# OpenDriveLab/ThinkTwice

Hardware: AMD Instinct MI355X
Metric: frames/sec forward (4-cam+LiDAR, thinktwice.py cfg) (higher is better)
Workload: dtype bf16x3h; 1 GPU; forward_inference thinktwice.py cfg: 8 frames x (2 sweeps x 4 cams x 448x896 + 65536-pt LiDAR), ResNet50+PAFPN+DepthNet+UNet+LSS splat, LidarNet, fusion, 5-stage decoder; parallelism=replicas x1 (no data-path collective), launch=eager launches, 3 batches in flight on alternating streams, batches_in_flight=3

## Files before the change

### thinktwice_amd/csrc/conv_choose.cpp

```cpp
#include <stdint.h>

#include "conv_choose.h"

namespace tt {
namespace {

bool aligned16(const void* p) { return (reinterpret_cast<uintptr_t>(p) & 15) == 0; }

void set_tile(ConvChoice* c, int family, int bn, int waves_m, int waves_n, int bkb, int stages) {
    c->family = family;
    c->bn = bn;
    c->waves_m = waves_m;
    c->waves_n = waves_n;
    c->bkb = bkb;
    c->stages = stages;
}

bool choose_h2(const ConvArgs& a, ConvChoice* c) {
    if (a.gather || a.m_dev || a.ws || a.pixel_shuffle2 || a.Cin % 64 != 0 || a.KH * a.KW > 31 || a.K < 64) return false;
    static const bool pipe = env_flag("TT_H2_PIPE", true);
    if (pipe && a.Cout % 128 == 0 && a.K >= 1152) set_tile(c, CONV_H2_PIPE, 128, 4, 1, 128, 32);
    else if (a.Cout > 64) set_tile(c, CONV_H2, 128, 4, 2, 128, 32);
    else set_tile(c, CONV_H2, 64, 8, 1, 128, 33);
    return true;
}

bool choose_small(const ConvArgs& a, ConvChoice* c) {
    if (a.gather || a.m_dev || a.M > 4096) return false;
    if ((long long)div_up(a.M, 32) * div_up(a.Cout, 32) > 4096) return false;
    set_tile(c, CONV_SMALL, 32, 1, 1, 32, 1);
    return true;
}

int tail_split_rows(const ConvArgs& a) {
    if (a.Cout % 256 != 0) return 0;
    const int tiles_m = div_up(a.M, 256), tiles_n = a.Cout / 256;
    const long long T = (long long)tiles_m * tiles_n;
    const int rounds = (int)((T + kNumCU - 1) / kNumCU);
    const int last = (int)(T - (long long)kNumCU * (rounds - 1));
    if (rounds < 2 || rounds > 8 || last > kNumCU / 4) return 0;
    const int peel = div_up(last, tiles_n);
    return peel < tiles_m ? tiles_m - peel : 0;
}

bool choose_x3_splitk(const ConvArgs& a, bool assume_ws, ConvChoice* c) {
    if (a.gather || a.m_dev || a.M < 512 || a.M > 8192 || a.Cout < 64 || a.KH * a.KW > 32) return false;
    if (a.Cin % 32 != 0 || a.K < 1024 || a.pixel_shuffle2) return false;
    const int tiles = div_up(a.M, 256) * div_up(a.Cout, 64);
    const int nk = a.K / 32;
    if (tiles >= 256) return false;
    int sp = 512 / tiles;
    if (sp > nk / 8) sp = nk / 8;
    if (sp > 16) sp = 16;
    if (sp < 2) return false;
    const int slices = div_up(nk, div_up(nk, sp));
    if (slices < 2 || (!assume_ws && a.ws_slices < slices)) return false;
    set_tile(c, CONV_GLDS, 64, 8, 1, 128, 2);
    c->x3 = true;
    c->splits = sp;
    c->slices = slices;
    return true;
}

bool choose_sp_runs(const ConvArgs& a, ConvChoice* c) {
    if (!a.gather || a.row_perm || a.KH != 1 || a.KW != 27) return false;
    if (a.stride != 1) return false;
    if (a.Cin % 32 != 0 || a.Cin > 128 || a.M < 2048 || a.pixel_shuffle2) return false;
    if ((a.in_cstride & 3) || (a.in_coff & 3)) return false;
    if (a.Cout == 32) set_tile(c, CONV_SP_RUNS, 32, 8, 1, 128, 2);
    else if (a.Cout == 64) set_tile(c, CONV_SP_RUNS, 64, 8, 1, 128, 2);
    else if (a.Cout == 128) set_tile(c, CONV_SP_RUNS, 128, 4, 2, 128, 2);
    else return false;
    c->gather = c->x3 = true;
    return true;
}

bool x3_pipe_ok(const ConvArgs& a, int bn) {
    return !(a.gather || a.m_dev || (bn != 256 && bn != 128) || a.Cout % bn != 0 || a.Cin % 32 != 0 || a.KH * a.KW > 31 || a.K < 64);
}

bool choose_x3(const ConvArgs& a, ConvChoice* c) {
    c->x3 = true;
    if (a.gather) {
        if (choose_sp_runs(a, c)) return true;
        const bool cin_ok = a.Cin >= 16 && (a.Cin & (a.Cin - 1)) == 0;
        if (!cin_ok || a.M < 2048 || a.Cout < 16 || a.Cout > 128) return false;
        set_tile(c, CONV_GLDS, a.Cout <= 32 ? 32 : (a.Cout <= 64 ? 64 : 128), 8, 1, 128, 2);
        c->gather = true;
        return true;
    }
    if (a.m_dev || a.M < 2048 || a.KH * a.KW > 32) return false;
    if (a.Cin % 32 != 0 || a.K < 64) return false;
    const bool apair = (a.flags & 32) != 0;
    if (apair && (a.in_coff % 16 != 0 || a.in_cstride % 16 != 0)) return false;
    c->apair = apair;
    if (a.Cout < 64) {
        if (a.Cout > 32 || a.Cout < 8) return false;
        if (!apair && a.M < (1 << 16)) return false;
        set_tile(c, CONV_GLDS, 32, 8, 1, 128, 2);
        return true;
    }
    const int tiles_m = div_up(a.M, 256);
    auto cost = [&](int bn, double rate) {
        const long long tiles = (long long)tiles_m * div_up(a.Cout, bn);
        return (double)((tiles + kNumCU - 1) / kNumCU) * bn / rate;
    };
    const bool wide = a.Cout % 256 == 0 || a.Cout > 512;
    const int main_rows = tail_split_rows(a);
    auto cost256 = [&]() {
        if (!main_rows) return cost(256, 1.0);
        const long long tn = a.Cout / 256;
        const long long main_tiles = (long long)main_rows * tn, tail_tiles = (long long)(tiles_m - main_rows) * tn * 4;
        return (double)((main_tiles + kNumCU - 1) / kNumCU) * 256 / 1.0 + (double)((tail_tiles + kNumCU - 1) / kNumCU) * 64 / 0.63;
    };
    const double c256 = wide ? cost256() : 1e30;
    const double c128 = a.Cout > 64 ? cost(128, (a.K >= 1152 && a.Cout % 128 == 0) ? 0.95 : 0.85) : 1e30;
    const double c64 = cost(64, 0.63);
    const int bn = (c256 <= c128 && c256 <= c64) ? 256 : (c128 <= c64 ? 128 : 64);
    static const bool pipe = env_flag("TT_X3_PIPE", true);
    if (pipe && a.K >= 1152 && bn != 64 && x3_pipe_ok(a, bn)) {
        static const bool run3 = env_flag("TT_X3_RUN3", true);
        const bool runs = run3 && a.KW == 3 && a.KH <= 5 && a.stride == 1 && a.dil == 1 && a.pad == 1 && a.OH == a.H && a.OW == a.W &&
                          (a.N == 1 || a.in_nstride == (long long)a.H * a.W * a.in_cstride);
        set_tile(c, runs ? CONV_X3_RUN3 : CONV_X3_PIPE, bn, 4, 1, 128, 23);
    } else if (bn == 256) {
        set_tile(c, CONV_GLDS, 256, 4, 2, 128, 23);
    } else {
        set_tile(c, CONV_GLDS, bn, 8, 1, 128, 2);
    }
    if (bn == 256) c->main_rows = main_rows;
    return true;
}

bool choose_glds(const ConvArgs& a, int dtype, ConvChoice* c) {
    constexpr int min_tiles = 2;
    if (a.gather) {
        const bool cin_ok = a.Cin >= 16 && (a.Cin & (a.Cin - 1)) == 0;
        if (dtype == TT_F32 || !cin_ok || a.M < 2048 || a.Cout < 16 || a.Cout > 128) return false;
        if (a.Cout <= 32) set_tile(c, CONV_GLDS, 32, 8, 1, 128, 2);
        else if (a.Cout <= 64) set_tile(c, CONV_GLDS, 64, 8, 1, 128, 2);
        else set_tile(c, CONV_GLDS, 128, 4, 2, 128, 2);
        c->gather = true;
        return true;
    }
    if (a.m_dev || a.M < 2048 || a.Cout < 64 || a.KH * a.KW > 32) return false;
    if (dtype == TT_F32) {
        if (a.Cin % 16 != 0 || div_up(a.K, 16) < min_tiles) return false;
        if (a.Cout > 64) set_tile(c, CONV_GLDS, 128, 4, 2, 64, 3);
        else set_tile(c, CONV_GLDS, 64, 8, 1, 64, 3);
        return true;
    }
    if (a.Cin % 32 != 0 || div_up(a.K, 32) < min_tiles) return false;
    if (a.Cout > 64) {
        const long long tiles256 = (long long)div_up(a.M, 256) * (a.Cout / 256);
        if (a.Cout % 256 == 0 && tiles256 >= 200) {
            if (a.Cin % 64 == 0) {
                set_tile(c, CONV_GLDS, 256, 2, 4, 128, 2);
                c->main_rows = tail_split_rows(a);
            } else {
                set_tile(c, CONV_GLDS, 256, 2, 4, 64, 3);
            }
        } else if (a.K <= 512) {
            set_tile(c, CONV_GLDS, 128, 2, 2, 64, 3);
        } else {
            set_tile(c, CONV_GLDS, 128, 4, 2, 64, 3);
        }
        return true;
    }
    if (a.Cin % 64 == 0) set_tile(c, CONV_GLDS, 64, 8, 1, 128, 2);
    else set_tile(c, CONV_GLDS, 64, 8, 1, 64, 3);
    return true;
}

int choose_igemm(const ConvArgs& a, int dtype, bool ws, bool assume_ws, ConvChoice* c) {
    if (a.Cout > 64) set_tile(c, CONV_IGEMM, 128, 2, 2, 64, 2);
    else if (a.Cout > 32) set_tile(c, CONV_IGEMM, 64, 2, 2, 64, 2);
    else set_tile(c, CONV_IGEMM, 32, 4, 1, 64, 2);
    if (dtype != TT_F32) c->bkb = 128;
    c->gather = a.gather != nullptr;
    const int tiles = div_up(a.M, 128) * div_up(a.Cout, c->bn);
    const int nk = div_up(a.K, c->bkb / (dtype == TT_F32 ? 4 : 2));
    if (ws && !a.m_dev && tiles < 128 && nk >= 8) {
        int sp = div_up(512, tiles);
        if (sp > nk / 2) sp = nk / 2;
        if (sp > 64) sp = 64;
        c->splits = sp < 1 ? 1 : sp;
    }
    if (c->splits <= 1) return 0;
    c->slices = c->splits;
    if (!assume_ws) {
        c->slices = 0;
        if (a.ws_slices > 0) {
            const int eff = div_up(nk, div_up(nk, c->splits));
            TT_REQUIRE(a.ws_slices >= eff, "tt_conv2d_fwd: split-K workspace holds %d slices, %d needed", a.ws_slices, eff);
            c->slices = eff;
        }
    }
    return 0;
}

}

int conv_choose(const ConvArgs& a, const ConvFacts& f, ConvChoice* c) {
    *c = ConvChoice{};
    c->splits = 1;
    const bool ws = a.ws || f.assume_ws;
    if (f.weight_h2) {
        TT_REQUIRE(aligned16(f.weight_h2), "tt_conv2d_fwd: weight_h2 must be 16-byte aligned");
        TT_REQUIRE(choose_h2(a, c), "tt_conv2d_fwd: weight_h2 layer outside the h2 kernel's contract (Cin=%d KH*KW=%d)", a.Cin,
                   a.KH * a.KW);
        return 0;
    }
    TT_REQUIRE(!f.out2 || a.vec_epi, "tt_conv2d_fwd: out2 needs the vector epilogue (aligned channel counts)");
    TT_REQUIRE(!f.res1_up || a.vec_epi, "tt_conv2d_fwd: an upsampled res1 needs the vector epilogue (aligned channel counts)");
    TT_REQUIRE(!f.res1_f32 || (a.vec_epi && a.res_vec), "tt_conv2d_fwd: an f32 res1 needs the vector epilogue and aligned residual rows");
    TT_REQUIRE(!(f.dtype == TT_F32 && a.out_dtype != TT_F32 && a.res1) || (a.vec_epi && a.res_vec),
               "tt_conv2d_fwd: a 16-bit output of an f32 layer with a residual needs the vector epilogue");
    if (a.flags & (32 | 64)) {
        TT_REQUIRE(a.vec_epi && aligned16(f.weight_x3) && a.K % 16 == 0,
                   "tt_conv2d_fwd: in_pair / out_pair need the vector epilogue and a 16-byte aligned weight_x3");
        TT_REQUIRE(choose_x3(a, c), "tt_conv2d_fwd: pair-format layer outside the LDS-DMA bf16x3 kernel's contract (M=%d Cin=%d Cout=%d)",
                   a.M, a.Cin, a.Cout);
        return 0;
    }
    if (!ws && !f.out2 && !f.res1_up && !f.res1_f32 && choose_small(a, c)) return 0;
    const bool x3 = f.weight_x3 && f.dtype == TT_F32;
    if (ws && x3 && a.K % 16 == 0 && aligned16(f.weight_x3) && choose_x3_splitk(a, f.assume_ws, c)) return 0;
    if (!ws && x3) {
        TT_REQUIRE(aligned16(f.weight_x3) && a.K % 16 == 0, "tt_conv2d_fwd: weight_x3 needs 16-byte alignment and K %% 16 == 0 (K = %d)",
                   a.K);
        if (choose_x3(a, c)) return 0;
        *c = ConvChoice{};
        c->splits = 1;
    }
    if (!ws && choose_glds(a, f.dtype, c)) return 0;
    return choose_igemm(a, f.dtype, ws, f.assume_ws, c);
}

ConvChoice conv_tail_choice(const ConvChoice& c) {
    ConvChoice t{};
    set_tile(&t, CONV_GLDS, 64, 8, 1, 128, 2);
    t.x3 = c.x3;
    t.apair = c.apair;
    t.splits = 1;
    return t;
}

void conv_label(const ConvChoice& c, int dtype, char* out, size_t bytes) {
    const char* tn = dtype == TT_F32 ? "float" : "16-bit";
    const char* pre = c.apair ? " pre-split A" : "";
    const char* tail = c.main_rows > 0 ? " + tail" : "";
    switch (c.family) {
        case CONV_H2: snprintf(out, bytes, "conv_h2_kernel<%d, %d, %d, %d, %d>", c.bn, c.waves_m, c.waves_n, c.stages / 10, c.stages % 10); break;
        case CONV_H2_PIPE: snprintf(out, bytes, "conv_h2_pipe_kernel"); break;
        case CONV_SMALL: snprintf(out, bytes, "conv_small_kernel"); break;
        case CONV_SP_RUNS: snprintf(out, bytes, "sp_conv_runs_kernel<%d, %d, %d>", c.bn / (32 * c.waves_n), c.waves_m, c.waves_n); break;
        case CONV_X3_PIPE: snprintf(out, bytes, "conv_x3_pipe_kernel<%s>%s%s", c.bn == 128 ? "4, 1, 128" : "4, 1", pre, tail); break;
        case CONV_X3_RUN3: snprintf(out, bytes, "conv_x3_run3_kernel<%d>%s%s", c.bn, pre, tail); break;
        case CONV_GLDS:
            snprintf(out, bytes, "conv_igemm_glds_kernel<%s, %d, %d, %d, %d, %d, %s, %s>%s%s", tn, c.bn, c.waves_m, c.waves_n, c.bkb,
                     c.stages, c.gather ? "true" : "false", c.x3 ? "true" : "false", pre, c.splits > 1 ? " split-K" : tail);
            break;
        default: snprintf(out, bytes, "conv_igemm_kernel<%s, 128, %d>%s", tn, c.bn, c.splits > 1 ? " split-K" : ""); break;
    }
}

}
```

### thinktwice_amd/csrc/conv_choose.h

```cpp
#pragma once
#include <stddef.h>

#include "tt_common.h"

namespace tt {

struct ConvArgs {
    const void* in;
    const void* weight;
    void* out;
    const float* scale;
    const float* shift;
    const float* shift_n;
    const void* res1;
    const void* res2;
    const int* gather;
    const int* m_dev;
    const int* row_perm;
    const unsigned* row_mask;
    float* ws;
    long long in_nstride, out_nstride;
    int N, H, W, Cin, in_cstride, in_coff;
    int Cout, KH, KW, stride, pad, dil;
    int OH, OW, out_cstride, out_coff;
    int pixel_shuffle2, shift_n_mod;
    int res1_cstride, res1_coff, res2_cstride, res2_coff;
    int act, out_dtype;
    int M, K;
    int cin_fast;
    int out_fast;
    int vec_epi;
    int res_vec;
    int splits;
    int tiles_n;
    int m_begin;
    int ws_slices;
    int flags;
    int res1_up_h, res1_up_w;
    float* out2;
    int out2_cstride, out2_coff;
    long long* trace;
};

enum ConvFamily {
    CONV_H2,
    CONV_H2_PIPE,
    CONV_SMALL,
    CONV_SP_RUNS,
    CONV_X3_PIPE,
    CONV_X3_RUN3,
    CONV_GLDS,
    CONV_IGEMM,
};

struct ConvFacts {
    int dtype;
    const void* weight_x3;
    const void* weight_h2;
    bool out2, res1_up, res1_f32;
    bool assume_ws;
};

struct ConvChoice {
    int family;
    int bn;
    int waves_m, waves_n, bkb, stages;
    bool gather, x3, apair;
    int main_rows;
    int splits;
    int slices;
};

int conv_choose(const ConvArgs& a, const ConvFacts& f, ConvChoice* c);
ConvChoice conv_tail_choice(const ConvChoice& c);
void conv_label(const ConvChoice& c, int dtype, char* out, size_t bytes);

}
```

### thinktwice_amd/csrc/conv_common.h

```cpp
#pragma once
#include <type_traits>
#include "conv_choose.h"

namespace tt {
extern thread_local char g_conv_kernel[96];
extern long long* g_conv_trace;


typedef float f32x16 __attribute__((ext_vector_type(16)));
typedef __bf16 bf16x8 __attribute__((ext_vector_type(8)));
typedef _Float16 f16x8 __attribute__((ext_vector_type(8)));

template <typename T> struct Mfma;
template <> struct Mfma<float> {
    __device__ static __forceinline__ void run(const uint4& a, const uint4& b, f32x16& c) {
        c = __builtin_amdgcn_mfma_f32_32x32x2f32(__uint_as_float(a.x), __uint_as_float(b.x), c, 0, 0, 0);
        c = __builtin_amdgcn_mfma_f32_32x32x2f32(__uint_as_float(a.y), __uint_as_float(b.y), c, 0, 0, 0);
        c = __builtin_amdgcn_mfma_f32_32x32x2f32(__uint_as_float(a.z), __uint_as_float(b.z), c, 0, 0, 0);
        c = __builtin_amdgcn_mfma_f32_32x32x2f32(__uint_as_float(a.w), __uint_as_float(b.w), c, 0, 0, 0);
    }
};
template <> struct Mfma<uint16_t> {
    __device__ static __forceinline__ void run(const uint4& a, const uint4& b, f32x16& c) {
        c = __builtin_amdgcn_mfma_f32_32x32x16_bf16(__builtin_bit_cast(bf16x8, a),
// ... 89 lines not shown
            v[4] += u.b.x; v[5] += u.b.y; v[6] += u.b.z; v[7] += u.b.w;
        } else {
            v[0] += u.x; v[1] += u.y; v[2] += u.z; v[3] += u.w;
        }
    };
    auto add_rv = [&](float (&v)[CO], const RV& u) {
        if constexpr (sizeof(T) == 2 && CO == 8) {
            const uint32_t w[4] = {u.x, u.y, u.z, u.w};
#pragma unroll
            for (int e = 0; e < 4; ++e) {
                float a, b;
                Pair16<T>::unpack(w[e], a, b);
                v[2 * e] += a; v[2 * e + 1] += b;
            }
        } else if constexpr (sizeof(T) == 2) {
            const uint32_t w[2] = {u.x, u.y};
#pragma unroll
            for (int e = 0; e < 2; ++e) {
                float a, b;
                Pair16<T>::unpack(w[e], a, b);
                v[2 * e] += a; v[2 * e + 1] += b;
            }
        } else {
            add_rvf(v, u);
        }
    };
    const bool r1_f32 = EXT && sizeof(T) == 2 && (p.flags & 128) != 0;
    const bool fast_act = (act == TT_ACT_NONE || act == TT_ACT_RELU);
    const bool r1_up = EXT && p.res1_up_w > 0;
    auto res1_row = [&](int m) -> long long {
        if (!r1_up) return (long long)m;
        const int n = m / ohw, rem = m - n * ohw;
        const int oh = rem / p.OW, ow = rem - oh * p.OW;
        return ((long long)n * p.res1_up_h + (oh * p.res1_up_h) / p.OH) * p.res1_up_w + (ow * p.res1_up_w) / p.OW;
    };
    auto out_offset = [&](int m, int cc, int& n) -> long long {
        if (p.out_fast) {
            if (has_sn) n = m / ohw;
            return (long long)m * p.out_cstride + p.out_coff + cc;
        }
        n = m / ohw;
        const int rem = m - n * ohw;
        int oh = rem / p.OW, ow = rem - oh * p.OW;
        int OWo = p.OW;
        if (p.pixel_shuffle2) {
            oh = 2 * oh + (q >> 1);
            ow = 2 * ow + (q & 1);
            OWo = 2 * p.OW;
        }
        return (long long)n * p.out_nstride + ((long long)oh * OWo + ow) * p.out_cstride + p.out_coff + cc;
    };
    const bool nt_store = (p.flags & 16) != 0;
    auto store_row = [&](long long o, const float (&v)[CO]) {
        if constexpr (CO == 4) {
            typedef float f4v __attribute__((ext_vector_type(4)));
            if (nt_store) __builtin_nontemporal_store(f4v{v[0], v[1], v[2], v[3]}, reinterpret_cast<f4v*>(reinterpret_cast<float*>(p.out) + o));
            else *reinterpret_cast<float4*>(reinterpret_cast<float*>(p.out) + o) = make_float4(v[0], v[1], v[2], v[3]);
        } else if (sizeof(T) == 4 && (p.flags & 64)) {
            uint4 hi, lo;
            uint32_t* hp = reinterpret_cast<uint32_t*>(&hi);
            uint32_t* lp = reinterpret_cast<uint32_t*>(&lo);
#pragma unroll
            for (int e = 0; e < 4; ++e) {
                const uint32_t h = pack_bf16x2(v[2 * e], v[2 * e + 1]);
                hp[e] = h;
                lp[e] = pack_bf16x2(v[2 * e] - __uint_as_float(h << 16), v[2 * e + 1] - __uint_as_float(h & 0xffff0000u));
            }
            float* g = reinterpret_cast<float*>(p.out) + (o & ~15ll) + ((o & 8) ? 4 : 0);
            *reinterpret_cast<uint4*>(g) = hi;
            *reinterpret_cast<uint4*>(g + 8) = lo;
        } else {
            uint4 pk;
            if constexpr (sizeof(T) == 2) {
                pk.x = Pair16<T>::pack(v[0], v[1]);
                pk.y = Pair16<T>::pack(v[2], v[3]);
                pk.z = Pair16<T>::pack(v[4], v[5]);
                pk.w = Pair16<T>::pack(v[6], v[7]);
            } else if (p.out_dtype == TT_F16) {
                pk.x = pack_f16x2(v[0], v[1]);
                pk.y = pack_f16x2(v[2], v[3]);
                pk.z = pack_f16x2(v[4], v[5]);
                pk.w = pack_f16x2(v[6], v[7]);
            } else {
                pk.x = pack_bf16x2(v[0], v[1]);
                pk.y = pack_bf16x2(v[2], v[3]);
                pk.z = pack_bf16x2(v[4], v[5]);
                pk.w = pack_bf16x2(v[6], v[7]);
            }
            *reinterpret_cast<uint4*>(reinterpret_cast<uint16_t*>(p.out) + o) = pk;
        }
    };
    float* const out2 = (EXT && p.out2) ? p.out2 + p.out2_coff + co : nullptr;
    auto store_row2 = [&](long long row, const float (&v)[CO]) {
        typedef float f4v __attribute__((ext_vector_type(4)));
        float* q2 = out2 + row * p.out2_cstride;
#pragma unroll
        for (int e = 0; e < CO; e += 4)
            __builtin_nontemporal_store(f4v{v[e], v[e + 1], v[e + 2], v[e + 3]}, reinterpret_cast<f4v*>(q2 + e));
    };
    const int cc = col_ok ? co : 0;
#pragma unroll
    for (int i = 0; i < TM; ++i) {
        const int mb = m0 + wm * WTM + i * 32;
        const int last_row = (mb + 31 < Mlim ? mb + 31 : Mlim - 1);
        const int img = mb / ohw;
        const bool one_image = (img == last_row / ohw);
        const bool sn_folded = has_sn && one_image;
        const bool sn_loop = has_sn && !sn_folded;
        float shb[TN];
#pragma unroll
        for (int j = 0; j < TN; ++j) shb[j] = sh[j];
        if (sn_folded) {
            const int nimg = img % p.shift_n_mod;
#pragma unroll
            for (int j = 0; j < TN; ++j) {
                const int cj = n0 + wn * WTN + j * 32 + (lane & 31);
                if (cj < p.Cout) shb[j] += p.shift_n[(long long)nimg * cout_real + cj % cout_real];
            }
        }
        stage_scaled<TN, WTN>(sC, acc[i], sc, shb, lane);
        const bool full_block = (mb + 32 <= Mlim) && (n0 + wn * WTN + WTN <= p.Cout);
        const bool out_linear = p.out_fast || (one_image && !p.pixel_shuffle2);
        const long long obase = (p.out_fast ? 0 : (long long)img * (p.out_nstride - (long long)ohw * p.out_cstride)) +
                                p.out_coff + co;
        if (fast_act && rvec && out_linear && !sn_loop && !has_r2 && full_block) {
            auto hot = [&](auto mode_c) {
                constexpr int RM = decltype(mode_c)::value;
                constexpr bool R1 = RM != 0;
                using R1T = typename std::conditional<RM == 2, RVF, RV>::type;
                using RES = typename std::conditional<RM == 2, float, T>::type;
                constexpr int PG = (sizeof(R1T) > 16 && NPASS > 4) ? 4 : (NPASS > 8 ? 8 : NPASS);
#pragma unroll
                for (int g0 = 0; g0 < NPASS; g0 += PG) {
                    R1T r1[R1 ? PG : 1];
                    int mrow[PG];
#pragma unroll
                    for (int q = 0; q < PG; ++q) {
                        const int m = mb + (g0 + q) * rpp + row_in_pass;
                        mrow[q] = p.row_perm ? p.row_perm[m] : m;
                    }
                    if constexpr (R1) {
#pragma unroll
                        for (int q = 0; q < PG; ++q)
                            r1[q] = *reinterpret_cast<const R1T*>(reinterpret_cast<const RES*>(p.res1) +
                                                                 res1_row(mrow[q]) * p.res1_cstride + p.res1_coff + co);
                    }
#pragma unroll
                    for (int q = 0; q < PG; ++q) {
                        const int rl = (g0 + q) * rpp + row_in_pass;
                        const int mr = mrow[q];
                        float v[CO];
#pragma unroll
                        for (int e = 0; e < CO; e += 4) {
                            const float4 t0 = *reinterpret_cast<const float4*>(sC + rl * LDC + col_l + e);
                            v[e] = t0.x; v[e + 1] = t0.y; v[e + 2] = t0.z; v[e + 3] = t0.w;
                        }
                        if constexpr (RM == 2) add_rvf(v, r1[q]);
                        else if constexpr (RM == 1) add_rv(v, r1[q]);
                        if (act == TT_ACT_RELU) {
#pragma unroll
                            for (int e = 0; e < CO; ++e) v[e] = v[e] > 0.f ? v[e] : 0.f;
                        }
                        store_row((long long)mr * p.out_cstride + obase, v);
                        if (out2) store_row2(mr, v);
                    }
                }
            };
            if (!has_r1) hot(std::integral_constant<int, 0>{});
            else if (EXT && sizeof(T) == 2 && r1_f32) {
                if constexpr (EXT && sizeof(T) == 2) hot(std::integral_constant<int, 2>{});
            } else hot(std::integral_constant<int, 1>{});
        } else {
#pragma unroll 1
            for (int pass = 0; pass < NPASS; ++pass) {
                const int rl = pass * rpp + row_in_pass;
                const int m = mb + rl;
                if (m >= Mlim || !col_ok) continue;
                float v[CO];
#pragma unroll
                for (int e = 0; e < CO; e += 4) {
                    const float4 t0 = *reinterpret_cast<const float4*>(sC + rl * LDC + col_l + e);
                    v[e] = t0.x; v[e + 1] = t0.y; v[e + 2] = t0.z; v[e + 3] = t0.w;
                }
                int n = 0;
                const int mo = p.row_perm ? p.row_perm[m] : m;
                const long long o = out_offset(mo, co, n);
                if (sn_loop) {
                    const float* sn = p.shift_n + (long long)(n % p.shift_n_mod) * cout_real + co;
#pragma unroll
                    for (int e = 0; e < CO; ++e) v[e] += sn[e];
                }
#pragma unroll
                for (int which = 0; which < 2; ++which) {
                    const void* rb = which ? p.res2 : p.res1;
                    if (!rb) continue;
                    const T* rp = reinterpret_cast<const T*>(rb) +
                                  (which ? (long long)mo : res1_row(mo)) * (which ? p.res2_cstride : p.res1_cstride) +
                                  (which ? p.res2_coff : p.res1_coff) + co;
                    if (which == 0 && r1_f32) {
                        const float* rf = reinterpret_cast<const float*>(rb) + res1_row(mo) * p.res1_cstride + p.res1_coff + co;
#pragma unroll
                        for (int e = 0; e < CO; ++e) v[e] += rf[e];
                    } else if (rvec) {
                        add_rv(v, *reinterpret_cast<const RV*>(rp));
                    } else {
#pragma unroll
                        for (int e = 0; e < CO; ++e) v[e] += Elem<T>::ld(rp + e);
                    }
                }
#pragma unroll
                for (int e = 0; e < CO; ++e) v[e] = apply_act(v[e], act);
                store_row(o, v);
                if (out2) store_row2(mo, v);
            }
        }
    }
}

template <typename T, int TM, int TN, int WTM, int WTN, bool EXT = (sizeof(T) == 4)>
__device__ __forceinline__ void conv_epilogue(const ConvArgs& p, f32x16 (&acc)[TM][TN], unsigned char* smem,
                                              int wave, int lane, int wm, int wn, int m0, int n0, int Mlim) {
    const int cout_real = p.pixel_shuffle2 ? (p.Cout >> 2) : p.Cout;
    const int ohw = p.OH * p.OW;
    if (p.act == 99) return;
    if (p.ws) {
#pragma unroll
        for (int j = 0; j < TN; ++j) {
            const int col = n0 + wn * WTN + j * 32 + (lane & 31);
            if (col >= p.Cout) continue;
#pragma unroll
            for (int i = 0; i < TM; ++i)
#pragma unroll
                for (int r = 0; r < 16; ++r) {
                    const int m = m0 + wm * WTM + i * 32 + (r & 3) + 8 * (r >> 2) + 4 * (lane >> 5);
                    if (m < Mlim) {
                        if (p.ws_slices > 0) p.ws[((long long)blockIdx.y * p.M + m) * p.Cout + col] = acc[i][j][r];
                        else unsafeAtomicAdd(p.ws + (long long)m * p.Cout + col, acc[i][j][r]);
                    }
                }
        }
        return;
    }
    float* sC = reinterpret_cast<float*>(smem) + wave * (32 * (WTN + 4));
    __syncthreads();
    if (p.vec_epi) {
        if (p.out_dtype == TT_F32 && !(p.flags & 64))
            conv_epilogue_vec<T, 4, TM, TN, WTM, WTN, EXT>(p, acc, sC, lane, wm, wn, m0, n0, Mlim);
        else
            conv_epilogue_vec<T, 8, TM, TN, WTM, WTN, EXT>(p, acc, sC, lane, wm, wn, m0, n0, Mlim);
        return;
    }
    constexpr int LDC = WTN + 4;
    const int act = p.act;
    float sc[TN], sh[TN];
    load_scale_shift<TN, WTN>(p, sc, sh, lane, wn, n0);
#pragma unroll
    for (int i = 0; i < TM; ++i) {
        stage_scaled<TN, WTN>(sC, acc[i], sc, sh, lane);
#pragma unroll 1
        for (int idx = lane; idx < 32 * WTN; idx += 64) {
            const int rl = idx / WTN, cl = idx - rl * WTN;
            const int m = m0 + wm * WTM + i * 32 + rl;
            const int col = n0 + wn * WTN + cl;
            if (m >= Mlim || col >= p.Cout) continue;
            int co = col, q = 0;
            if (p.pixel_shuffle2) {
                q = col / cout_real;
                co = col - q * cout_real;
            }
            float v = sC[rl * LDC + cl];
            const int n = m / ohw;
            const int mo = p.row_perm ? p.row_perm[m] : m;
            long long o;
            if (p.out_fast) {
                o = (long long)mo * p.out_cstride + p.out_coff + co;
            } else {
                const int rem = m - n * ohw;
                int oh = rem / p.OW, ow = rem - oh * p.OW;
                int OWo = p.OW;
                if (p.pixel_shuffle2) {
                    oh = 2 * oh + (q >> 1);
                    ow = 2 * ow + (q & 1);
                    OWo = 2 * p.OW;
                }
                o = (long long)n * p.out_nstride + ((long long)oh * OWo + ow) * p.out_cstride + p.out_coff + co;
            }
            if (p.shift_n) v += p.shift_n[(n % p.shift_n_mod) * cout_real + co];
            if (p.res1)
                v += Elem<T>::ld(reinterpret_cast<const T*>(p.res1) + (long long)mo * p.res1_cstride + p.res1_coff + co);
            if (p.res2)
                v += Elem<T>::ld(reinterpret_cast<const T*>(p.res2) + (long long)mo * p.res2_cstride + p.res2_coff + co);
            v = apply_act(v, act);
            if (p.out_dtype == TT_F32)
                reinterpret_cast<float*>(p.out)[o] = v;
            else
                store16(p.out, o, v, p.out_dtype);
            if (p.out2) p.out2[(long long)mo * p.out2_cstride + p.out2_coff + co] = v;
        }
    }
}

int launch_conv_h2(const ConvChoice& c, ConvArgs& a, hipStream_t st);
int launch_conv_small(ConvArgs& a, int dtype, hipStream_t st);
int launch_sp_conv_runs(const ConvChoice& c, ConvArgs& a, hipStream_t st);
int launch_conv_x3_pipe(const ConvChoice& c, ConvArgs& a, hipStream_t st);
int launch_conv_glds(const ConvChoice& c, ConvArgs& a, int dtype, hipStream_t st);

}
```

### thinktwice_amd/csrc/conv_igemm.hip

```cpp
#include <stdlib.h>

#include "conv_common.h"

namespace tt {

template <typename T, int BM, int BN, int WAVES_M, int WAVES_N, bool GATHER, int KX = 1>
__global__ __launch_bounds__(256) void conv_igemm_kernel(const ConvArgs p) {
    constexpr int VEC = Elem<T>::kVec;
    constexpr int BKB = ((sizeof(T) == 4) ? 64 : 128) * KX;
    constexpr int BK = BKB / (int)sizeof(T);
    constexpr int VPR = BKB / 16;
    constexpr int ROWB = BKB + 16;
    constexpr int NVA = (BM * VPR + 255) / 256;
    constexpr int NVB = (BN * VPR + 255) / 256;
    constexpr int WTM = BM / WAVES_M, WTN = BN / WAVES_N;
    constexpr int TM = WTM / 32, TN = WTN / 32;
    static_assert(WAVES_M * WAVES_N == 4, "4 waves");

    extern __shared__ __attribute__((aligned(16))) unsigned char smem[];
    const int nbuf = (p.K > BK) ? 2 : 1;
    unsigned char* sA = smem;
    unsigned char* sB = smem + nbuf * BM * ROWB;

    const int tid = threadIdx.x;
// ... 62 lines not shown
    uint4 ra[NVA], rb[NVB];

    auto load_tile = [&](int kt) {
        const int k0 = kt * BK;
        int tap_u = 0, ci_u = 0, kh_u = 0, kw_u = 0;
        if (p.cin_fast) {
            tap_u = k0 / p.Cin;
            ci_u = k0 - tap_u * p.Cin;
            kh_u = tap_u / p.KW;
            kw_u = tap_u - kh_u * p.KW;
        }
#pragma unroll
        for (int i = 0; i < NVA; ++i) {
            int kh, kw, ci;
            const int k = k0 + a_vc[i] * VEC;
            if (p.cin_fast) {
                kh = kh_u; kw = kw_u; ci = ci_u + a_vc[i] * VEC;
            } else {
                const int tap = k / p.Cin;
                ci = k - tap * p.Cin;
                kh = tap / p.KW;
                kw = tap - kh * p.KW;
            }
            if (GATHER) {
                int j = -1;
                if (p.cin_fast) {
                    j = jn[i];
                    const int kn = k0 + BK;
                    jn[i] = (a_ok[i] && kn < p.K) ? p.gather[a_base[i] + kn / p.Cin] : -1;
                } else if (a_ok[i] && (k < p.K)) {
                    j = p.gather[a_base[i] + kh * p.KW + kw];
                }
                if (j >= 0) {
                    const T* src = in + (long long)j * p.in_cstride + p.in_coff + ci;
                    ra[i] = *reinterpret_cast<const uint4*>(src);
                } else {
                    ra[i] = make_uint4(0, 0, 0, 0);
                }
            } else {
                const int ih = a_h0[i] + kh * p.dil;
                const int iw = a_w0[i] + kw * p.dil;
                const bool ok = a_ok[i] && (k < p.K) && ih >= 0 && ih < p.H && iw >= 0 && iw < p.W;
                if (ok) {
                    const T* src = in + a_base[i] + ((long long)ih * p.W + iw) * p.in_cstride + ci;
                    ra[i] = *reinterpret_cast<const uint4*>(src);
                } else {
                    ra[i] = make_uint4(0, 0, 0, 0);
                }
            }
        }
#pragma unroll
        for (int i = 0; i < NVB; ++i) {
            const int k = k0 + b_vc[i] * VEC;
            if (b_ok[i] && k < p.K) {
                rb[i] = *reinterpret_cast<const uint4*>(wgt + (long long)(n0 + b_row[i]) * p.K + k);
            } else {
                rb[i] = make_uint4(0, 0, 0, 0);
            }
        }
    };
    auto store_tile = [&](int buf) {
#pragma unroll
        for (int i = 0; i < NVA; ++i)
            if (tid + 256 * i < BM * VPR)
                *reinterpret_cast<uint4*>(sA + (buf * BM + a_row[i]) * ROWB + a_vc[i] * 16) = ra[i];
#pragma unroll
        for (int i = 0; i < NVB; ++i)
            if (tid + 256 * i < BN * VPR)
                *reinterpret_cast<uint4*>(sB + (buf * BN + b_row[i]) * ROWB + b_vc[i] * 16) = rb[i];
    };

    f32x16 acc[TM][TN];
    zero_acc(acc);

    if (GATHER && p.cin_fast) {
#pragma unroll
        for (int i = 0; i < NVA; ++i)
            jn[i] = (a_ok[i] && kt0 * BK < p.K) ? p.gather[a_base[i] + (kt0 * BK) / p.Cin] : -1;
    }
    load_tile(kt0);
    store_tile(0);
    __syncthreads();

    const int frag_off = (lane & 31) * ROWB + (lane >> 5) * 16;
    for (int kt = kt0; kt < nk; ++kt) {
        const int buf = (kt - kt0) & 1;
        if (kt + 1 < nk) load_tile(kt + 1);
        const unsigned char* tA = sA + (buf * BM + wm * WTM) * ROWB + frag_off;
        const unsigned char* tB = sB + (buf * BN + wn * WTN) * ROWB + frag_off;
#pragma unroll
        for (int kc = 0; kc < BKB / 32; ++kc) {
            uint4 fa[TM], fb[TN];
#pragma unroll
            for (int i = 0; i < TM; ++i)
                fa[i] = *reinterpret_cast<const uint4*>(tA + i * 32 * ROWB + kc * 32);
#pragma unroll
            for (int j = 0; j < TN; ++j)
                fb[j] = *reinterpret_cast<const uint4*>(tB + j * 32 * ROWB + kc * 32);
#pragma unroll
            for (int i = 0; i < TM; ++i)
#pragma unroll
                for (int j = 0; j < TN; ++j) Mfma<T>::run(fa[i], fb[j], acc[i][j]);
        }
        if (kt + 1 < nk) store_tile(buf ^ 1);
        __syncthreads();
    }

    conv_epilogue<T, TM, TN, WTM, WTN>(p, acc, smem, wave, lane, wm, wn, m0, n0, Mlim);
}

template <typename T>
__global__ __launch_bounds__(256) void splitk_finalize_kernel(const ConvArgs p) {
    const long long t = (long long)blockIdx.x * blockDim.x + threadIdx.x;
    if (t >= (long long)p.M * p.Cout) return;
    const int m = (int)(t / p.Cout), col = (int)(t % p.Cout);
    const int cout_real = p.pixel_shuffle2 ? (p.Cout >> 2) : p.Cout;
    int co = col, q = 0;
    if (p.pixel_shuffle2) { q = col / cout_real; co = col - q * cout_real; }
    const int ohw = p.OH * p.OW;
    const int n = m / ohw;
    const int rem = m - n * ohw;
    int oh = rem / p.OW, ow = rem - oh * p.OW, OWo = p.OW;
    if (p.pixel_shuffle2) { oh = 2 * oh + (q >> 1); ow = 2 * ow + (q & 1); OWo = 2 * p.OW; }
    const long long o = (long long)n * p.out_nstride + ((long long)oh * OWo + ow) * p.out_cstride + p.out_coff + co;
    float acc = p.ws[t];
    for (int sl = 1; sl < p.ws_slices; ++sl) acc += p.ws[(long long)sl * p.M * p.Cout + t];
    float v = acc * (p.scale ? p.scale[co] : 1.f) + (p.shift ? p.shift[co] : 0.f);
    if (p.shift_n) v += p.shift_n[(n % p.shift_n_mod) * cout_real + co];
    if (p.res1) v += Elem<T>::ld(reinterpret_cast<const T*>(p.res1) + (long long)m * p.res1_cstride + p.res1_coff + co);
    if (p.res2) v += Elem<T>::ld(reinterpret_cast<const T*>(p.res2) + (long long)m * p.res2_cstride + p.res2_coff + co);
    v = apply_act(v, p.act);
    if (p.out_dtype == TT_F32) reinterpret_cast<float*>(p.out)[o] = v;
    else store16(p.out, o, v, p.out_dtype);
}

template <typename T, int BM, int BN, int WAVES_M, int WAVES_N, bool GATHER, int KX = 1>
static int launch_conv(const ConvChoice& c, ConvArgs& a, hipStream_t st) {
    constexpr int BKB = ((sizeof(T) == 4) ? 64 : 128) * KX;
    constexpr int BK = BKB / (int)sizeof(T);
    constexpr int ROWB = BKB + 16;
    const int tiles_m = div_up(a.M, BM);
    a.tiles_n = div_up(a.Cout, BN);
    a.cin_fast = (a.Cin % BK == 0) ? 1 : 0;
    constexpr int WTN_ = BN / WAVES_N;
    size_t smem = (size_t)((a.K > BK) ? 2 : 1) * (BM + BN) * ROWB;
    const size_t epi = (size_t)4 * 32 * (WTN_ + 4) * 4;
    if (smem < epi) smem = epi;
    auto kern = conv_igemm_kernel<T, BM, BN, WAVES_M, WAVES_N, GATHER, KX>;
    const int tiles = tiles_m * a.tiles_n;
    a.splits = c.splits;
    if (a.splits <= 1) a.ws = nullptr;
    if (a.ws) a.ws_slices = c.slices;
    size_t mx = (size_t)2 * (BM + BN) * ROWB;
    if (mx < epi) mx = epi;
    if (mx > 48 * 1024 && lds_opt_in(reinterpret_cast<const void*>(kern), mx, "conv_igemm_kernel")) return -1;
    hipLaunchKernelGGL(kern, dim3((unsigned)tiles, (unsigned)a.splits), dim3(256), smem, st, a);
    return 1;
}

template <typename T, bool GATHER>
static int launch_igemm2(const ConvChoice& c, ConvArgs& a, hipStream_t st) {
    if (c.bn == 128 && c.waves_m == 2 && c.waves_n == 2) return launch_conv<T, 128, 128, 2, 2, GATHER>(c, a, st);
    if (c.bn == 64 && c.waves_m == 2 && c.waves_n == 2) return launch_conv<T, 128, 64, 2, 2, GATHER>(c, a, st);
    if (c.bn == 32 && c.waves_m == 4 && c.waves_n == 1) return launch_conv<T, 128, 32, 4, 1, GATHER>(c, a, st);
    TT_REQUIRE(false, "tt_conv2d_fwd: no conv_igemm_kernel for a %d-wide tile of %d x %d waves", c.bn, c.waves_m, c.waves_n);
}

static int launch_conv_igemm(const ConvChoice& c, ConvArgs& a, int dtype, hipStream_t st) {
    if (dtype == TT_F32) return a.gather ? launch_igemm2<float, true>(c, a, st) : launch_igemm2<float, false>(c, a, st);
    if (dtype == TT_F16) return a.gather ? launch_igemm2<f16_t, true>(c, a, st) : launch_igemm2<f16_t, false>(c, a, st);
    return a.gather ? launch_igemm2<uint16_t, true>(c, a, st) : launch_igemm2<uint16_t, false>(c, a, st);
}

static void launch_splitk_finalize(const ConvArgs& a, int dtype, hipStream_t st) {
    const dim3 grid((unsigned)div_up((long long)a.M * a.Cout, 256));
    if (dtype == TT_F32) hipLaunchKernelGGL(splitk_finalize_kernel<float>, grid, dim3(256), 0, st, a);
    else if (dtype == TT_F16) hipLaunchKernelGGL(splitk_finalize_kernel<f16_t>, grid, dim3(256), 0, st, a);
    else hipLaunchKernelGGL(splitk_finalize_kernel<uint16_t>, grid, dim3(256), 0, st, a);
}

}

using namespace tt;

static int conv2d_prepare(const tt_conv_desc* d, ConvArgs& a, ConvFacts& f) {
    TT_REQUIRE(d && d->in && d->weight && d->out, "tt_conv2d_fwd: null pointer");
    TT_REQUIRE(d->dtype == TT_F32 || d->dtype == TT_BF16 || d->dtype == TT_F16, "tt_conv2d_fwd: bad dtype %d", d->dtype);
    TT_REQUIRE(d->out_dtype == TT_F32 || d->out_dtype == d->dtype ||
                   (d->dtype == TT_F32 && (d->out_dtype == TT_F16 || d->out_dtype == TT_BF16) && !d->res2),
               "tt_conv2d_fwd: out_dtype must be TT_F32, the operand dtype, or (f32 operands, at most res1) a 16-bit type "
               "(got %d for dtype %d)", d->out_dtype, d->dtype);
    TT_REQUIRE(!d->res1_f32 || (d->weight_h2 && d->res1),
               "tt_conv2d_fwd: res1_f32 goes with an h2 layer's res1 (the other 16-bit kernels read residuals of their operand type)");
    TT_REQUIRE(d->dtype == TT_F32 || d->weight_h2 || (!d->out2 && d->res1_up_w <= 0),
               "tt_conv2d_fwd: out2 / res1_up_* exist in the f32-operand kernels and the h2 kernel only");
    TT_REQUIRE(!d->weight_h2 || (d->dtype == TT_F16 && !d->gather_idx && !d->splitk_ws && !d->pixel_shuffle2),
               "tt_conv2d_fwd: weight_h2 goes with dense TT_F16 operands (no split-K workspace, no pixel shuffle)");
    TT_REQUIRE(!d->out2 || (!d->splitk_ws && !d->pixel_shuffle2 && !d->gather_idx && d->out2_cstride % 4 == 0 &&
                            d->out2_coff % 4 == 0 && (reinterpret_cast<uintptr_t>(d->out2) & 15) == 0),
               "tt_conv2d_fwd: out2 needs a dense row-linear layer and 16-byte aligned rows");
    const int vec = d->dtype == TT_F32 ? 4 : 8;
    TT_REQUIRE(d->Cin > 0 && d->Cin % vec == 0 && d->in_cstride % vec == 0 && d->in_coff % vec == 0,
               "tt_conv2d_fwd: Cin=%d in_cstride=%d in_coff=%d must be multiples of %d (pad channels)",
               d->Cin, d->in_cstride, d->in_coff, vec);
    TT_REQUIRE((reinterpret_cast<uintptr_t>(d->in) & 15) == 0 &&
                   (reinterpret_cast<uintptr_t>(d->weight) & 15) == 0,
               "tt_conv2d_fwd: in/weight must be 16-byte aligned");
    TT_REQUIRE(d->N > 0 && d->H > 0 && d->W > 0 && d->Cout > 0 && d->KH > 0 && d->KW > 0 &&
                   d->stride > 0 && d->dil > 0 && d->OH > 0 && d->OW > 0,
               "tt_conv2d_fwd: bad geometry");
    TT_REQUIRE(!d->pixel_shuffle2 || d->Cout % 4 == 0, "tt_conv2d_fwd: pixel_shuffle2 needs Cout%%4==0");
    a.in = d->in; a.weight = d->weight; a.out = d->out;
    a.scale = d->scale; a.shift = d->shift; a.shift_n = d->shift_n;
    a.res1 = d->res1; a.res2 = d->res2;
    a.gather = d->gather_idx; a.m_dev = d->m_dev;
    a.row_perm = d->gather_idx ? d->row_perm : nullptr;
    a.row_mask = d->gather_idx ? d->row_mask : nullptr;
    TT_REQUIRE(!a.row_perm == !a.row_mask, "tt_conv2d_fwd: row_perm and row_mask come together");
    a.ws = d->splitk_ws;
    a.ws_slices = d->splitk_ws ? d->splitk_slices : 0;
    TT_REQUIRE(!d->gather_idx || (d->H == 1 && d->W == 1 && d->OH == 1 && d->OW == 1 && d->KH == 1 &&
                                  !d->pixel_shuffle2),
               "tt_conv2d_fwd: gather mode wants H=W=OH=OW=KH=1, KW=taps");
    a.N = d->N; a.H = d->H; a.W = d->W; a.Cin = d->Cin; a.in_cstride = d->in_cstride; a.in_coff = d->in_coff;
    a.in_nstride = d->in_nstride ? d->in_nstride : (long long)d->H * d->W * d->in_cstride;
    a.Cout = d->Cout; a.KH = d->KH; a.KW = d->KW; a.stride = d->stride; a.pad = d->pad; a.dil = d->dil;
    a.OH = d->OH; a.OW = d->OW; a.out_cstride = d->out_cstride; a.out_coff = d->out_coff;
    const long long def_on = (long long)d->OH * d->OW * d->out_cstride * (d->pixel_shuffle2 ? 4 : 1);
    a.out_nstride = d->out_nstride ? d->out_nstride : def_on;
    a.pixel_shuffle2 = d->pixel_shuffle2;
    a.shift_n_mod = d->shift_n_mod > 0 ? d->shift_n_mod : 1;
    a.res1_cstride = d->res1_cstride; a.res1_coff = d->res1_coff;
    a.res2_cstride = d->res2_cstride; a.res2_coff = d->res2_coff;
    a.act = d->act; a.out_dtype = d->out_dtype;
    a.out2 = d->out2; a.out2_cstride = d->out2_cstride; a.out2_coff = d->out2_coff;
    a.res1_up_h = d->res1_up_h; a.res1_up_w = d->res1_up_w;
    TT_REQUIRE((d->res1_up_h > 0) == (d->res1_up_w > 0) && (d->res1_up_w <= 0 || (d->res1 && !d->gather_idx && !d->splitk_ws &&
                                                                                 !d->pixel_shuffle2)),
               "tt_conv2d_fwd: res1_up_h / res1_up_w come together, with a dense layer's res1");
    a.M = d->N * d->OH * d->OW;
    a.K = d->KH * d->KW * d->Cin;
    a.out_fast = (!d->pixel_shuffle2 && a.out_nstride == (long long)d->OH * d->OW * d->out_cstride) ? 1 : 0;
    TT_REQUIRE(!(d->pixel_shuffle2 && (d->res1 || d->res2)),
               "tt_conv2d_fwd: residuals are not supported with pixel_shuffle2");
    a.tiles_n = 1; a.cin_fast = 0; a.m_begin = 0;
    a.trace = g_conv_trace;
    a.flags = 16;
    if (d->in_pair || d->out_pair) {
        TT_REQUIRE(d->dtype == TT_F32 && d->out_dtype == TT_F32 && d->weight_x3 && !d->gather_idx && !d->splitk_ws && !d->pixel_shuffle2,
                   "tt_conv2d_fwd: in_pair / out_pair go with dense bf16x3 layers (f32 containers, weight_x3, no split-K workspace)");
        TT_REQUIRE(!d->out_pair || (!d->res1 && !d->res2 && !d->shift_n && d->Cout % 16 == 0 && d->out_cstride % 16 == 0 &&
                                    d->out_coff % 16 == 0 && (reinterpret_cast<uintptr_t>(d->out) & 63) == 0),
                   "tt_conv2d_fwd: out_pair needs Cout / out_cstride / out_coff multiples of 16, a 64-byte aligned output and no "
                   "residual / per-image shift");
        if (d->in_pair) a.flags |= 32;
        if (d->out_pair) a.flags |= 64;
    }
    if (d->res1_f32) a.flags |= 128;
    {
        const int co_vec = (d->out_dtype == TT_F32 && !d->out_pair) ? 4 : 8;
        const int osz = d->out_dtype == TT_F32 ? 4 : 2;
        const int cr = d->pixel_shuffle2 ? d->Cout / 4 : d->Cout;
        bool ok = (cr % co_vec == 0) && (d->out_cstride % co_vec == 0) && (d->out_coff % co_vec == 0) &&
                  (a.out_nstride % co_vec == 0) && ((reinterpret_cast<uintptr_t>(d->out) & 15) == 0);
        (void)osz;
        a.vec_epi = ok ? 1 : 0;
        auto res_ok = [&](const void* r, int cs, int co_) {
            return !r || ((cs % co_vec == 0) && (co_ % co_vec == 0) && ((reinterpret_cast<uintptr_t>(r) & 15) == 0));
        };
        a.res_vec = (res_ok(d->res1, d->res1_cstride, d->res1_coff) && res_ok(d->res2, d->res2_cstride, d->res2_coff)) ? 1 : 0;
    }
    f.dtype = d->dtype;
    f.weight_x3 = d->weight_x3;
    f.weight_h2 = d->weight_h2;
    f.out2 = d->out2 != nullptr;
    f.res1_up = d->res1_up_w > 0;
    f.res1_f32 = d->res1_f32 != 0;
    f.assume_ws = false;
    return 0;
}

extern "C" int tt_conv2d_fwd(const tt_conv_desc* d, void* stream) {
    ConvArgs a;
    ConvFacts f;
    ConvChoice c;
    if (const int r = conv2d_prepare(d, a, f)) return r;
    if (const int r = conv_choose(a, f, &c)) return r;
    hipStream_t st = (hipStream_t)stream;
    const bool pair = d->in_pair || d->out_pair;
    const char* what = "tt_conv2d_fwd";
    int r;
    if (c.x3) a.weight = d->weight_x3;
    switch (c.family) {
        case CONV_H2:
        case CONV_H2_PIPE:
            a.weight = d->weight_h2;
            what = "tt_conv2d_fwd(h2)";
            r = launch_conv_h2(c, a, st);
            break;
        case CONV_SMALL:
            what = "tt_conv2d_fwd(small)";
            r = launch_conv_small(a, d->dtype, st);
            break;
        case CONV_SP_RUNS:
            what = "tt_conv2d_fwd(glds x3)";
            r = launch_sp_conv_runs(c, a, st);
            break;
        case CONV_X3_PIPE:
        case CONV_X3_RUN3:
            what = pair ? "tt_conv2d_fwd(glds x3, pair)" : "tt_conv2d_fwd(glds x3)";
            r = launch_conv_x3_pipe(c, a, st);
            break;
        case CONV_GLDS:
            what = !c.x3 ? "tt_conv2d_fwd(glds)" : c.splits > 1 ? "tt_conv2d_fwd(glds x3 split-K)" : pair ? "tt_conv2d_fwd(glds x3, pair)" : "tt_conv2d_fwd(glds x3)";
            if (c.splits > 1) a.ws_slices = c.slices;
            r = launch_conv_glds(c, a, d->dtype, st);
            break;
        default:
            a.row_perm = nullptr;
            a.row_mask = nullptr;
            r = launch_conv_igemm(c, a, d->dtype, st);
            break;
    }
    if (r < 0) return r;
    conv_label(c, d->dtype, g_conv_kernel, sizeof(g_conv_kernel));
    if (c.main_rows > 0) {
        ConvArgs t = a;
        t.m_begin = c.main_rows * 256;
        if (launch_conv_glds(conv_tail_choice(c), t, d->dtype, st) < 0) return -1;
    }
    if (c.splits > 1) launch_splitk_finalize(a, d->dtype, st);
    return check_launch(what);
}

extern "C" int tt_conv2d_splitk_slices(const tt_conv_desc* d) {
    ConvArgs a;
    ConvFacts f;
    ConvChoice c;
    if (conv2d_prepare(d, a, f)) return 0;
    if (d->in_pair || d->out_pair || d->weight_h2 || d->res1_up_w > 0) return 0;
    f.assume_ws = true;
    if (conv_choose(a, f, &c)) return 0;
    return c.splits > 1 ? c.slices : 0;
}

extern "C" int tt_conv2d_plan(const tt_conv_desc* d, char* label, int label_bytes) {
    ConvArgs a;
    ConvFacts f;
    ConvChoice c;
    if (const int r = conv2d_prepare(d, a, f)) return r;
    if (const int r = conv_choose(a, f, &c)) return r;
    TT_REQUIRE(label && label_bytes > 0, "tt_conv2d_plan: no room for the label");
    conv_label(c, d->dtype, label, (size_t)label_bytes);
    return 0;
}
```

Before: 104.2 frames/s.

## Add persistent LDS-resident-weight kernel for small-channel 27-tap sparse convs

Result: faster. 106.1 frames/s (median of 6 runs) (+1.8%).

```diff
diff --git a/thinktwice_amd/csrc/conv_choose.cpp b/thinktwice_amd/csrc/conv_choose.cpp
--- a/thinktwice_amd/csrc/conv_choose.cpp
+++ b/thinktwice_amd/csrc/conv_choose.cpp
@@ -62,6 +62,15 @@
     return true;
 }
 
+bool choose_sp_runs_l2(const ConvArgs& a, ConvChoice* c) {
+    if (!a.gather || a.row_perm || a.KH != 1 || a.KW != 27 || a.pixel_shuffle2 || a.M < kSpL2MinRows) return false;
+    if ((a.Cin != 16 && a.Cin != 32) || (a.Cout != 16 && a.Cout != 32 && a.Cout != 64)) return false;
+    if ((a.in_cstride & 3) || (a.in_coff & 3) || !aligned16(a.in) || !a.vec_epi || a.out_dtype != TT_F32) return false;
+    set_tile(c, CONV_SP_RUNS_L2, 32, 8, 1, a.Cin * 4, 1);
+    c->gather = c->x3 = true;
+    return true;
+}
+
 bool choose_sp_runs(const ConvArgs& a, ConvChoice* c) {
     if (!a.gather || a.row_perm || a.KH != 1 || a.KW != 27) return false;
     if (a.stride != 1) return false;
@@ -82,6 +91,7 @@
 bool choose_x3(const ConvArgs& a, ConvChoice* c) {
     c->x3 = true;
     if (a.gather) {
+        if (choose_sp_runs_l2(a, c)) return true;
         if (choose_sp_runs(a, c)) return true;
         const bool cin_ok = a.Cin >= 16 && (a.Cin & (a.Cin - 1)) == 0;
         if (!cin_ok || a.M < 2048 || a.Cout < 16 || a.Cout > 128) return false;
@@ -254,6 +264,7 @@
         case CONV_H2: snprintf(out, bytes, "conv_h2_kernel<%d, %d, %d, %d, %d>", c.bn, c.waves_m, c.waves_n, c.stages / 10, c.stages % 10); break;
         case CONV_H2_PIPE: snprintf(out, bytes, "conv_h2_pipe_kernel"); break;
         case CONV_SMALL: snprintf(out, bytes, "conv_small_kernel"); break;
+        case CONV_SP_RUNS_L2: snprintf(out, bytes, "sp_conv_runs_l2_kernel<%d>", c.bkb / 4); break;
         case CONV_SP_RUNS: snprintf(out, bytes, "sp_conv_runs_kernel<%d, %d, %d>", c.bn / (32 * c.waves_n), c.waves_m, c.waves_n); break;
         case CONV_X3_PIPE: snprintf(out, bytes, "conv_x3_pipe_kernel<%s>%s%s", c.bn == 128 ? "4, 1, 128" : "4, 1", pre, tail); break;
         case CONV_X3_RUN3: snprintf(out, bytes, "conv_x3_run3_kernel<%d>%s%s", c.bn, pre, tail); break;
diff --git a/thinktwice_amd/csrc/conv_choose.h b/thinktwice_amd/csrc/conv_choose.h
--- a/thinktwice_amd/csrc/conv_choose.h
+++ b/thinktwice_amd/csrc/conv_choose.h
@@ -46,12 +46,15 @@
     CONV_H2,
     CONV_H2_PIPE,
     CONV_SMALL,
+    CONV_SP_RUNS_L2,
     CONV_SP_RUNS,
     CONV_X3_PIPE,
     CONV_X3_RUN3,
     CONV_GLDS,
     CONV_IGEMM,
 };
+
+constexpr int kSpL2MinRows = 16384;
 
 struct ConvFacts {
     int dtype;
diff --git a/thinktwice_amd/csrc/conv_common.h b/thinktwice_amd/csrc/conv_common.h
--- a/thinktwice_amd/csrc/conv_common.h
+++ b/thinktwice_amd/csrc/conv_common.h
@@ -415,6 +415,7 @@
 
 int launch_conv_h2(const ConvChoice& c, ConvArgs& a, hipStream_t st);
 int launch_conv_small(ConvArgs& a, int dtype, hipStream_t st);
+int launch_sp_conv_l2(const ConvChoice& c, ConvArgs& a, hipStream_t st);
 int launch_sp_conv_runs(const ConvChoice& c, ConvArgs& a, hipStream_t st);
 int launch_conv_x3_pipe(const ConvChoice& c, ConvArgs& a, hipStream_t st);
 int launch_conv_glds(const ConvChoice& c, ConvArgs& a, int dtype, hipStream_t st);
diff --git a/thinktwice_amd/csrc/conv_igemm.hip b/thinktwice_amd/csrc/conv_igemm.hip
--- a/thinktwice_amd/csrc/conv_igemm.hip
+++ b/thinktwice_amd/csrc/conv_igemm.hip
@@ -388,6 +388,10 @@
             what = "tt_conv2d_fwd(small)";
             r = launch_conv_small(a, d->dtype, st);
             break;
+        case CONV_SP_RUNS_L2:
+            what = "tt_conv2d_fwd(sp l2)";
+            r = launch_sp_conv_l2(c, a, st);
+            break;
         case CONV_SP_RUNS:
             what = "tt_conv2d_fwd(glds x3)";
             r = launch_sp_conv_runs(c, a, st);
diff --git a/thinktwice_amd/csrc/sp_conv_l2.hip b/thinktwice_amd/csrc/sp_conv_l2.hip
--- /dev/null
+++ b/thinktwice_amd/csrc/sp_conv_l2.hip
@@ -0,0 +1,146 @@
+#include "conv_lds_dma.h"
+
+namespace tt {
+
+namespace {
+constexpr int kL2Taps = 27;
+constexpr int kL2Waves = 8;
+constexpr int kL2Slab = 32 * (32 + 4) * 4;
+}
+
+template <int CIN>
+__global__ __launch_bounds__(kL2Waves * 64, 1) void sp_conv_runs_l2_kernel(const ConvArgs p, const float* __restrict__ zp) {
+#if defined(__HIP_DEVICE_COMPILE__)
+    constexpr int KS = CIN / 16;
+    constexpr int ROWB = CIN * 4;
+    constexpr int WB = kL2Taps * 32 * ROWB;
+    constexpr int NP = WB / 1024;
+    constexpr int RPP = 1024 / ROWB, CPR = ROWB / 16;
+    static_assert(CIN == 16 || CIN == 32, "one or two k-steps");
+    static_assert(WB % 1024 == 0, "whole DMA pieces");
+
+    extern __shared__ __attribute__((aligned(16))) unsigned char smem[];
+    const int tid = threadIdx.x, lane = tid & 63, wave = tid >> 6;
+    const int wave_s = __builtin_amdgcn_readfirstlane(wave);
+    const int n0 = (int)blockIdx.y * 32;
+    int Mlim = p.M;
+    if (p.m_dev) {
+        const int md = *p.m_dev;
+        Mlim = md < Mlim ? md : Mlim;
+    }
+    const int ngroups = (Mlim + 31) >> 5;
+    int first = (int)blockIdx.x * kL2Waves;
+    const int end = ngroups, stride = (int)gridDim.x * kL2Waves;
+    if (first >= end) return;
+    first += wave_s;
+
+    const float* __restrict__ in = reinterpret_cast<const float*>(p.in) + p.in_coff;
+    const float* __restrict__ wgt = reinterpret_cast<const float*>(p.weight);
+
+    {
+        const unsigned lds_base = (unsigned)(uintptr_t)(__attribute__((address_space(3))) unsigned char*)smem;
+        const int d_row = lane / CPR, d_pos = lane % CPR;
+        for (int i = wave_s; i < NP; i += kL2Waves) {
+            const int r = i * RPP + d_row;
+            const int t = r >> 5, n = r & 31;
+            const int nn = n0 + n < p.Cout ? n0 + n : p.Cout - 1;
+            dma_piece(wgt + (long long)nn * p.K + t * CIN + ((d_pos ^ swz<ROWB>(n)) << 2), lds_base + (unsigned)i * 1024u);
+        }
+    }
+    __builtin_amdgcn_s_waitcnt(0x0F70);
+    __syncthreads();
+
+    float* const sC = reinterpret_cast<float*>(smem + WB + wave * kL2Slab);
+    const unsigned kb = lane >> 5;
+    unsigned boff[KS];
+#pragma unroll
+    for (int ks = 0; ks < KS; ++ks) boff[ks] = frag_off<ROWB>(lane & 31, 4u * ks + kb);
+    constexpr unsigned LO = 32u;
+
+    auto load_ent = [&](int g, int (&e)[kL2Taps]) {
+        const int m = g * 32 + (lane & 31);
+        const bool live = g < end && m < Mlim;
+        const int* __restrict__ rb = p.gather + (long long)(live ? m : Mlim - 1) * kL2Taps;
+#pragma unroll
+        for (int t = 0; t < kL2Taps; ++t) e[t] = rb[t];
+#pragma unroll
+        for (int t = 0; t < kL2Taps; ++t) e[t] = live ? e[t] : -1;
+    };
+    auto load_a = [&](int ent, float4 (&a)[KS][2]) {
+        const float* __restrict__ row = ent >= 0 ? in + (long long)ent * p.in_cstride : zp;
+        const float4* __restrict__ s = reinterpret_cast<const float4*>(row) + 2 * kb;
+#pragma unroll
+        for (int ks = 0; ks < KS; ++ks) {
+            a[ks][0] = s[4 * ks];
+            a[ks][1] = s[4 * ks + 1];
+        }
+    };
+
+    int e[kL2Taps];
+    load_ent(first, e);
+    for (int g = first; g < end; g += stride) {
+        f32x16 acc[1][1];
+        zero_acc(acc);
+        float4 a[3][KS][2];
+        load_a(e[0], a[0]);
+        load_a(e[1], a[1]);
+        int en[kL2Taps];
+        load_ent(g + stride, en);
+#pragma unroll
+        for (int t = 0; t < kL2Taps; ++t) {
+            if (t + 2 < kL2Taps) load_a(e[t + 2], a[(t + 2) % 3]);
+            if (__builtin_amdgcn_ballot_w64(e[t] >= 0) == 0ull) continue;
+            const unsigned char* wt = smem + t * (32 * ROWB);
+#pragma unroll
+            for (int ks = 0; ks < KS; ++ks) {
+                const uint4 bh = *reinterpret_cast<const uint4*>(wt + boff[ks]);
+                const uint4 bl = *reinterpret_cast<const uint4*>(wt + (boff[ks] ^ LO));
+                const float4 r0 = a[t % 3][ks][0], r1 = a[t % 3][ks][1];
+                const float x[8] = {r0.x, r0.y, r0.z, r0.w, r1.x, r1.y, r1.z, r1.w};
+                uint32_t h[4], l[4];
+#pragma unroll
+                for (int q = 0; q < 4; ++q) {
+                    h[q] = pack_bf16x2(x[2 * q], x[2 * q + 1]);
+                    const float q0 = x[2 * q] - __uint_as_float(h[q] << 16);
+                    const float q1 = x[2 * q + 1] - __uint_as_float(h[q] & 0xffff0000u);
+                    l[q] = pack_bf16x2(q0, q1);
+                }
+                const uint4 ah = uint4{h[0], h[1], h[2], h[3]}, al = uint4{l[0], l[1], l[2], l[3]};
+                Mfma<uint16_t>::run(al, bh, acc[0][0]);
+                Mfma<uint16_t>::run(ah, bl, acc[0][0]);
+                Mfma<uint16_t>::run(ah, bh, acc[0][0]);
+            }
+        }
+        if (p.act != 99)
+            conv_epilogue_vec<float, 4, 1, 1, 32, 32, true>(p, acc, sC, lane, 0, 0, g * 32, n0, Mlim);
+#pragma unroll
+        for (int t = 0; t < kL2Taps; ++t) e[t] = en[t];
+    }
+#endif
+}
+
+template <int CIN>
+static int launch_l2(ConvArgs& a, hipStream_t st) {
+    constexpr size_t smem = (size_t)kL2Taps * 32 * CIN * 4 + (size_t)kL2Waves * kL2Slab;
+    static_assert(smem <= 160 * 1024, "the CU's LDS");
+    auto kern = sp_conv_runs_l2_kernel<CIN>;
+    const void* zp = zero_page("sp_conv_runs_l2_kernel");
+    if (!zp || lds_opt_in(reinterpret_cast<const void*>(kern), smem, "sp_conv_runs_l2_kernel")) return -1;
+    const int ncol = div_up(a.Cout, 32);
+    int gx = div_up(a.M, kL2Waves * 32);
+    if (gx > kNumCU / ncol) gx = kNumCU / ncol;
+    a.tiles_n = ncol;
+    a.splits = 1;
+    a.ws = nullptr;
+    a.m_begin = 0;
+    hipLaunchKernelGGL(kern, dim3((unsigned)gx, (unsigned)ncol), dim3(kL2Waves * 64), smem, st, a, reinterpret_cast<const float*>(zp));
+    return 1;
+}
+
+int launch_sp_conv_l2(const ConvChoice& c, ConvArgs& a, hipStream_t st) {
+    if (a.Cin == 32 && c.bkb == 128) return launch_l2<32>(a, st);
+    if (a.Cin == 16 && c.bkb == 64) return launch_l2<16>(a, st);
+    TT_REQUIRE(false, "tt_conv2d_fwd: no sp_conv_runs_l2_kernel for Cin = %d", a.Cin);
+}
+
+}
```
